# makgyver/rectorch

Hardware: AMD Instinct MI355X
Metric: MultiVAE train users/sec on ml-20m (synthetic, ml-20m-shaped) (higher is better)
Workload: dtype bf16

## Files before the change

### __graft_entry__.py

```python
import os
import subprocess
import sys

ROOT = os.path.dirname(os.path.abspath(__file__))
if ROOT not in sys.path:
    sys.path.insert(0, ROOT)


def build():
    from rectorch_amd import _lib
    path = _lib.build()
    assert os.path.exists(path)
    subprocess.check_call(["make", "-C", os.path.join(ROOT, "oracle"), "-s"])
    subprocess.check_call(["make", "-C", os.path.join(ROOT, "tests", "native"), "-s"])
    import rectorch_amd
    from rectorch_amd import nets, models, samplers, evaluation, metrics, parallel
    assert _lib.lib().rtx_abi_version() == 8


def smoke():
    import numpy as np
    import torch
    from scipy.sparse import csr_matrix
    from rectorch_amd.nets import MultiVAE_net
    from rectorch_amd.models import MultiVAE
    from rectorch_amd.samplers import DataSampler
    from rectorch_amd.utils import hash_state_dict
    from oracle import c_oracle

    assert torch.cuda.is_available(), "smoke() needs the MI355X"
    torch.cuda.set_device(0)
    I, H, L, B = 300, 64, 16, 24
    rng = np.random.default_rng(0)
    dense = (rng.random((B, I)) < 0.08).astype(np.float64)
    dense[3] = 0
    sd = hash_state_dict([I, H, L], [L, H, I], "vae", 7, bias_std=0.3)
    net = MultiVAE_net([L, H, I], dropout=0.5)
    net.load_state_dict({k: torch.from_numpy(v) for k, v in sd.items()})
    model = MultiVAE(net, beta=0.2, anneal_steps=0, numerics="fp32")
    smp = DataSampler(csr_matrix(dense), batch_size=B, shuffle=False)
    (rb,) = list(smp.iter_rows())
    mask = (rng.random((B, I)) >= 0.5).astype(np.uint8)
    eps = rng.standard_normal((B, L)).astype(np.float32)
    model._rtx.inject = (torch.from_numpy(mask).cuda(), torch.from_numpy(eps).cuda())
    loss = model._fused_step(rb, None, want_loss=True)
    params = [sd[k] for k in ["enc_layers.0.weight", "enc_layers.0.bias", "enc_layers.1.weight", "enc_layers.1.bias",
                              "dec_layers.0.weight", "dec_layers.0.bias", "dec_layers.1.weight", "dec_layers.1.bias"]]
# ... 17 lines not shown
```

### rectorch_amd/csrc/engine.hip

```cpp
#include "engine_internal.h"

int dev_alloc(rtx_engine* e, void** p, size_t bytes, bool zero)
{
    if (bytes == 0) bytes = 16;
    hipError_t rc = hipMalloc(p, bytes);
    if (rc != hipSuccess) {
        rtx_set_error("hipMalloc(%zu bytes) failed: %s", bytes, hipGetErrorString(rc));
        return RTX_ENOMEM;
    }
    if (e) e->allocs.push_back(*p);
    if (zero) {
        RTX_HIP(hipMemset(*p, 0, bytes));
        RTX_HIP(hipStreamSynchronize(nullptr));
    }
    return RTX_OK;
}

void dev_free(rtx_engine* e, void* p)
{
    if (!p) return;
    auto it = std::find(e->allocs.begin(), e->allocs.end(), p);
    if (it != e->allocs.end()) e->allocs.erase(it);
    (void)hipFree(p);
}
// ... 287 lines not shown
    const int Bp = rtx_pad_batch(B);
    static const rtx_step zero_step = {};
    if (!step) step = &zero_step;
    const int sample = training || e->gvae;
    int64_t in_chunks = 0;
    const bool sparse_in = l0 == 0 && l1 > 1 && sparse_in_ok(e, in, Bp, &in_chunks);
    if (l0 == 0) e->last_sparse_in = sparse_in;
    const bool gathered = e->gather_done;
    e->gather_done = false;
    if (e->join_fold && !(l0 == 0 && l1 > 1 && !sparse_in && gathered && e->bf16)) {
        e->join_fold = false;
        RTX_TRY(launch_hop_wait(e, st, 3, e->join_seq));
    }
    if (l0 == 0 && !sparse_in && !gathered) RTX_TRY(gather_batch(e, in, tg, B, training, step, st));
    for (int li = l0; li < l1; ++li) {
        Layer& l = e->L[li];
        if (li == e->NL - 1) {
            RtxGemm g = {};
            g.form = RTX_FORM_NT;
            g.A = l.A; g.B = l.Wsh; g.lda = l.inp; g.ldb = l.inp;
            g.k_slices = (int)((size_t)l.inp * e->esz / 128);
            g.splits = 1; g.C = logits; g.ldc = ldlog; g.bias = e->params[2 * li + 1];
            g.M_real = B; g.N_real = l.out;
            TIMED("gemm_logits");
            if (e->bf16 && !e->opt_nt_regstage) {
                g.tile_shape = (Bp % 512 == 0) ? RTX_DMA_512x128 : RTX_DMA_128x128;
                int bm, bn;
                rtx_gemm_dma_tile_dims(g.tile_shape, &bm, &bn);
                g.m_tiles = Bp / bm; g.n_tiles = l.outp / bn;
                if (want_lse && e->opt_lse_fuse) { g.lse_part = e->lse_part; g.lse_ld = e->lse_strips; }
                g.xcd_block = 1;
                RTX_TRY(rtx_gemm_dma_launch(g, RTX_EPI_BIAS_ROWS, st));
            } else {
                g.tile_shape = RTX_TILE_128x128;
                g.m_tiles = Bp / 128; g.n_tiles = l.outp / 128;
                if (want_lse && e->opt_lse_fuse) { g.lse_part = e->lse_part; g.lse_ld = e->lse_strips; }
                if (want_lse && logits16_on(e)) { g.C16 = l.D; g.ldc16 = l.outp; }
                RTX_TRY(rtx_gemm_launch(g, e->bf16 ? RTX_DT_BF16 : RTX_DT_F32, RTX_EPI_BIAS_ROWS, st));
            }
            break;
        }
        if (li == 0 && sparse_in) {
            RTX_TRY(ensure_in_chunks(e, in_chunks, st));
            RtxInChunksArgs c = {};
            c.in = *in; c.B = B; c.I = e->I; c.Iin = e->Iin;
            c.training = training; c.dropout_p = e->cfg.dropout_p;
            c.mask = step->dropout_mask; c.seed = step->seed; c.offset = step->offset;
            c.ent = e->in_ent; c.desc = e->in_desc; c.wsplit = e->in_wsplit; c.cap_chunks = e->in_cap_chunks;
            if (training) { c.target = *tg; c.tsum = e->tsum; c.X = (bf16_t*)l.A; c.ldx = l.inp; c.Bp = Bp; e->img_exact = false; }
            {
                TIMED("in_chunks");
                RTX_TRY(rtx_launch_in_chunks(c, st));
            }
            RtxSpmmInArgs a = {};
            a.ent = e->in_ent; a.desc = e->in_desc; a.wsplit = e->in_wsplit;
            a.B = B; a.Bp = Bp;
            a.W = (const bf16_t*)l.Wsh; a.ldw = l.inp; a.Kin = e->Iin;
            a.bias = e->params[2 * li + 1]; a.N_real = l.out; a.Np = l.outp; a.tanh_act = l.tanh_act;
            a.O32 = l.O32; a.R = (bf16_t*)e->L[li + 1].A; a.ones_col = 1;
            TIMED("spmm_in");
            RTX_TRY(rtx_launch_spmm_in(a, st));
            continue;
        }
        if (li > 0 && e->bf16 && e->opt_small_fwd && rtx_small_fwd_ok(l.inp)) {
            Layer& nx1 = e->L[li + 1];
            RtxSmallFwdArgs a = {};
            a.A = (const bf16_t*)l.A; a.W = (const bf16_t*)l.Wsh; a.lda = l.inp; a.ldw = l.inp; a.w_rows = l.outp;
            a.B = B; a.Bp = Bp; a.bias = e->params[2 * li + 1]; a.R = (bf16_t*)nx1.A;
// ... 592 lines not shown
```

### rectorch_amd/csrc/engine_api.hip

```cpp
#include "engine_internal.h"

extern "C" {

enum OptKind {
    OPT_BOOL,
    OPT_INT,
    OPT_CHECKED,
    OPT_COUNTER,
};
struct OptEntry {
    const char* key;
    OptKind kind;
    int rtx_engine::*member;
    int DpState::*dp_member;
};
static const OptEntry OPTIONS[] = {
    {"fuse_adam", OPT_BOOL, &rtx_engine::opt_fuse_adam},
    {"lse_fuse", OPT_BOOL, &rtx_engine::opt_lse_fuse},
    {"logits16", OPT_BOOL, &rtx_engine::opt_logits16},
    {"hop_values", OPT_BOOL, &rtx_engine::opt_hop_values},
    {"hop_kernels", OPT_BOOL, &rtx_engine::opt_hop_kernels},
    {"hop_fold", OPT_BOOL, &rtx_engine::opt_hop_fold},
    {"timing_calibrate", OPT_BOOL, &rtx_engine::opt_timing_calibrate},
    {"f32_dw_split", OPT_BOOL, &rtx_engine::opt_f32_dw_split},
    {"splitk_fwd", OPT_INT, &rtx_engine::opt_splitk_fwd},
    {"splitk_bwd", OPT_INT, &rtx_engine::opt_splitk_bwd},
    {"gather_scatter", OPT_BOOL, &rtx_engine::opt_gather_scatter},
    {"prefetch", OPT_BOOL, &rtx_engine::opt_prefetch},
    {"two_stream", OPT_BOOL, &rtx_engine::opt_two_stream},
    {"nt_regstage", OPT_BOOL, &rtx_engine::opt_nt_regstage},
    {"in_on_main", OPT_BOOL, &rtx_engine::opt_in_on_main},
    {"sparse_in", OPT_BOOL, &rtx_engine::opt_sparse_in},
    {"small_fwd", OPT_BOOL, &rtx_engine::opt_small_fwd},
    {"small_bwd", OPT_BOOL, &rtx_engine::opt_small_bwd},
    {"big_batch_tiles", OPT_BOOL, &rtx_engine::opt_big_batch_tiles},
    {"dw_side_pad", OPT_CHECKED, &rtx_engine::opt_dw_side_pad},
    {"dp_shard_min_elems", OPT_CHECKED, &rtx_engine::opt_dp_shard_min_elems},
    {"dp_one_comm", OPT_CHECKED, &rtx_engine::opt_dp_one_comm},
    {"dw_cfg", OPT_CHECKED, &rtx_engine::opt_dw_cfg},
    {"join_folds", OPT_COUNTER, &rtx_engine::st_join_folds},
    {"prefetch_hits", OPT_COUNTER, &rtx_engine::st_prefetch_hits},
    {"prefetch_issued", OPT_COUNTER, &rtx_engine::st_prefetch_issued},
    {"last_sparse_in", OPT_COUNTER, &rtx_engine::last_sparse_in},
    {"side_concurrent", OPT_COUNTER, &rtx_engine::side_concurrent},
    {"dp_collectives", OPT_COUNTER, nullptr, &DpState::st_collectives},
};
static const char* const OPTIONS_SET_ONLY = "hop_wrap, splitk, small_kw, small_waves";
static const char* const OPTIONS_GET_ONLY = "splitk, dp_bytes_all_reduce, dp_bytes_reduce_scatter, dp_bytes_all_gather, dp_two_comms";

static std::string option_keys(bool writable)
{
    std::string out;
    for (const OptEntry& o : OPTIONS)
        if (!writable || o.kind != OPT_COUNTER) out += std::string(o.key) + ", ";
    return out + (writable ? OPTIONS_SET_ONLY : OPTIONS_GET_ONLY);
}

static int set_checked(rtx_engine* e, const std::string& k, int32_t value, bool* handled)
{
    *handled = true;
    if (k == "dw_side_pad") e->opt_dw_side_pad = value > 0 ? value : 0;
    else if (k == "small_kw") rtx_small_set_kw(value);
    else if (k == "small_waves") rtx_small_set_waves(value);
// ... 197 lines not shown
```

### rectorch_amd/csrc/engine_internal.h

```cpp
#pragma once
#include "../../include/rectorch_hip.h"
#include "rtx_gemm.h"
#include "rtx_kernels.h"

#include <math.h>
#include <stdlib.h>
#include <string.h>
#include <sched.h>
#include <algorithm>
#include <chrono>
#include <map>
#include <string>
#include <vector>

const char* rtx_last_error_str();

struct Layer {
    int in = 0, out = 0, inp = 0, outp = 0;
    bool tanh_act = false;
    void* Wsh = nullptr;
    void* Wsh_alt = nullptr;
    void* WshT = nullptr;
    void* A = nullptr;
    float* O32 = nullptr;
// ... 85 lines not shown
    int opt_hop_values = 1;
    int n_cus = 256;
    int opt_f32_dw_split = 1;
    int opt_splitk_bwd = 0;
    int opt_splitk_fwd = 0;
    uint32_t* hopk_mem = nullptr;
    uint32_t hopk_seq = 0;
    bool join_pending = false, join_fold = false;
    uint32_t join_seq = 0;
    int opt_timing_calibrate = 0;
    int opt_dw_side_pad = 0;
    int opt_hop_fold = 1;
    int opt_hop_kernels = 0;
    uint32_t* hop_mem = nullptr;
    uint32_t hop_seq = 0;
    uint32_t hop_wrap = 0x7ffffff0u;
    int opt_fuse_adam = 1;
    int opt_dw_cfg = RTX_DW_64x128;
    int opt_dp_shard_min_elems = 1 << 20;
    uint32_t* loss_mailbox = nullptr;
    uint32_t loss_ticket = 0;
    int opt_dp_one_comm = 0;
    int opt_dw_cfg_set = 0;
    int opt_lse_fuse = 1;
    int opt_logits16 = 1;
    int opt_two_stream = 1;
    int opt_in_on_main = 1;
    int opt_sparse_in = 0;
    int opt_small_fwd = 1;
    int opt_small_bwd = 1;
    int opt_big_batch_tiles = 1;
    int last_sparse_in = 0;
    int opt_nt_regstage = 1;
    bool timing_all = false;
    std::map<std::string, int> timing_sites;
    std::map<std::string, long> timing_seen;
    std::map<std::string, TimingSite> sites;
    std::vector<hipEvent_t> event_pool;
    DpState dp;
};

struct ScopedTimer {
    rtx_engine* e;
    hipStream_t s;
    TimingSite* site = nullptr;
    hipEvent_t e0 = nullptr, e1 = nullptr;
    std::string name;
    ScopedTimer(rtx_engine* eng, const char* nm, hipStream_t st) : e(eng), s(st), name(nm)
    {
        const char* name = nm;
        if (!e->timing_all && e->timing_sites.empty()) return;
        if (!e->timing_all) {
            auto it = e->timing_sites.find(name);
            if (it == e->timing_sites.end()) return;
            if (it->second > 1 && (e->timing_seen[name]++ % it->second) != 0) return;
        }
        site = &e->sites[name];
        auto get = [&]() {
            hipEvent_t ev;
            if (!e->event_pool.empty()) {
                ev = e->event_pool.back();
                e->event_pool.pop_back();
            } else if (hipEventCreate(&ev) != hipSuccess) {
                ev = nullptr;
            }
            return ev;
// ... 82 lines not shown
```

### rectorch_amd/csrc/gemm.hip

```cpp
#include "rtx_gemm.h"
#include <type_traits>

typedef __attribute__((ext_vector_type(8))) __bf16 bf16x8_t;
typedef __attribute__((ext_vector_type(16))) float f32x16_t;

#define RTX_LDS_ROW_OF(KB) ((KB) + 16)

template <typename T> struct Mma;

template <> struct Mma<bf16_t> {
    static __device__ __forceinline__ void run(f32x16_t& acc, const uint4& a, const uint4& b)
    {
        acc = __builtin_amdgcn_mfma_f32_32x32x16_bf16(__builtin_bit_cast(bf16x8_t, a), __builtin_bit_cast(bf16x8_t, b),
                                                      acc, 0, 0, 0);
    }
};

template <> struct Mma<fp8_t> {
    static __device__ __forceinline__ void run(f32x16_t& acc, const uint4& a, const uint4& b)
    {
        const long a0 = (long)(((unsigned long)a.y << 32) | a.x), a1 = (long)(((unsigned long)a.w << 32) | a.z);
        const long b0 = (long)(((unsigned long)b.y << 32) | b.x), b1 = (long)(((unsigned long)b.w << 32) | b.z);
        acc = __builtin_amdgcn_mfma_f32_32x32x16_fp8_fp8(a0, b0, acc, 0, 0, 0);
        acc = __builtin_amdgcn_mfma_f32_32x32x16_fp8_fp8(a1, b1, acc, 0, 0, 0);
    }
};

template <> struct Mma<float> {
    static __device__ __forceinline__ void run(f32x16_t& acc, const uint4& a, const uint4& b)
    {
        acc = __builtin_amdgcn_mfma_f32_32x32x2f32(__builtin_bit_cast(float, a.x), __builtin_bit_cast(float, b.x), acc, 0, 0, 0);
        acc = __builtin_amdgcn_mfma_f32_32x32x2f32(__builtin_bit_cast(float, a.y), __builtin_bit_cast(float, b.y), acc, 0, 0, 0);
        acc = __builtin_amdgcn_mfma_f32_32x32x2f32(__builtin_bit_cast(float, a.z), __builtin_bit_cast(float, b.z), acc, 0, 0, 0);
        acc = __builtin_amdgcn_mfma_f32_32x32x2f32(__builtin_bit_cast(float, a.w), __builtin_bit_cast(float, b.w), acc, 0, 0, 0);
    }
};

template <int WM, int WN, int NB, int KB = 128> struct TileCfg {
    static constexpr int NT = WM * WN * 64;
    static constexpr int BM = WM * 64;
    static constexpr int BN = WN * NB * 32;
    static constexpr int LPR = KB / 16;
    static constexpr int RPP = NT / LPR;
    static constexpr int PA = BM / RPP;
    static constexpr int PB = BN / RPP;
    static constexpr int ROW = RTX_LDS_ROW_OF(KB);
    static constexpr int STAGE = (BM + BN) * ROW;
    static_assert(PA == 2 || PA == 4, "PA");
    static_assert(PB == 2 || PB == 4, "PB");
};

template <typename T, int EPI, int WM, int WN, int NB, int KB = 128, bool DEPTH3 = false>
__global__ __launch_bounds__(WM* WN * 64, KB == 64 ? 3 : ((WM * WN) / 4 > 2 ? (WM * WN) / 4 : 2)) void rtx_gemm_nt(const RtxGemm p)
{
    using Cfg = TileCfg<WM, WN, NB, KB>;
    constexpr int BM = Cfg::BM, BN = Cfg::BN, RPP = Cfg::RPP, PA = Cfg::PA, PB = Cfg::PB, STAGE = Cfg::STAGE;
    constexpr int RTX_LDS_ROW = Cfg::ROW, LPR_ST = Cfg::LPR;
    __shared__ __attribute__((aligned(16))) unsigned char smem[2 * STAGE];

    if (p.wait_word) rtx_fold_wait(p.wait_word, p.wait_seq);
    const int tid = threadIdx.x;
    const int lane = tid & 63, wave = tid >> 6;
    const int wm = wave / WN, wn = wave % WN;
    const int r = lane & 31, g = lane >> 5;

    int tm, tn, split;
    {
        const int L = blockIdx.x, xcd = L & 7, j = L >> 3;
        if (p.syrk_lower) {
            split = 0;
            const int patch = xcd + 8 * (j >> 6), within = j & 63;
            int pm = (int)((sqrtf(8.f * (float)patch + 1.f) - 1.f) * 0.5f);
            while ((pm + 1) * (pm + 2) / 2 <= patch) ++pm;
            while (pm * (pm + 1) / 2 > patch) --pm;
            const int pn = patch - pm * (pm + 1) / 2;
            tm = pm * 8 + (within & 7);
            tn = pn * 8 + (within >> 3);
            if (tm >= p.m_tiles || tn > tm) return;
        } else if (p.splits > 1) {
            const int tiles = p.m_tiles * p.n_tiles;
            split = xcd + 8 * (j / tiles);
            if (split >= p.splits) return;
            const int t = j % tiles;
            tm = t % p.m_tiles;
            tn = t / p.m_tiles;
        } else if (p.m_tiles <= p.n_tiles) {
            split = 0;
            tn = xcd + 8 * (j / p.m_tiles);
            tm = j % p.m_tiles;
            if (tn >= p.n_tiles) return;
        } else {
            split = 0;
            tm = xcd + 8 * (j / p.n_tiles);
            tn = j % p.n_tiles;
            if (tm >= p.m_tiles) return;
        }
    }
    const int k_sl = p.k_slices * (128 / KB);
    const int per = (k_sl + p.splits - 1) / p.splits;
    const int ks0 = split * per;
    const int ks1 = min(ks0 + per, k_sl);
    const int nk = ks1 - ks0;

    const size_t rowA = (size_t)p.lda * sizeof(T), rowB = (size_t)p.ldb * sizeof(T);
    const size_t kstA = p.a_slice_stride ? (size_t)p.a_slice_stride : (size_t)KB, kstB = p.b_slice_stride ? (size_t)p.b_slice_stride : (size_t)KB;
    const int st_row = tid / LPR_ST, st_ch = tid % LPR_ST;
    const unsigned char* gA = (const unsigned char*)p.A + ((size_t)tm * BM + st_row) * rowA + st_ch * 16;
    const unsigned char* gB = (const unsigned char*)p.B + ((size_t)tn * BN + st_row) * rowB + st_ch * 16;
    const int lds_a = st_row * RTX_LDS_ROW + st_ch * 16;
    const int lds_b = (BM + st_row) * RTX_LDS_ROW + st_ch * 16;

    uint4 ra0, ra1, ra2, ra3, rb0, rb1, rb2, rb3;
    uint4 sa0, sa1, sa2, sa3, sb0, sb1, sb2, sb3;
    f32x16_t acc[2][NB];
#pragma unroll
    for (int i = 0; i < 2; ++i)
#pragma unroll
        for (int j = 0; j < NB; ++j)
#pragma unroll
            for (int e = 0; e < 16; ++e) acc[i][j][e] = 0.f;

#define RTX_GL(R, X, q, base, row, ks) R##X##q = *(const uint4*)((base) + (size_t)(q) * RPP * (row) + (size_t)(ks) * ((row) == rowA ? kstA : kstB));
#define RTX_GLOAD(R, ks) {                                                  \
    RTX_GL(R, a, 0, gA, rowA, ks) RTX_GL(R, a, 1, gA, rowA, ks)             \
    if (PA == 4) { RTX_GL(R, a, 2, gA, rowA, ks) RTX_GL(R, a, 3, gA, rowA, ks) } \
    RTX_GL(R, b, 0, gB, rowB, ks) RTX_GL(R, b, 1, gB, rowB, ks)             \
    if (PB == 4) { RTX_GL(R, b, 2, gB, rowB, ks) RTX_GL(R, b, 3, gB, rowB, ks) } }
#define RTX_LS(R, X, q, off, st) *(uint4*)(smem + (st) * STAGE + (off) + (q) * RPP * RTX_LDS_ROW) = R##X##q;
#define RTX_LSTORE(R, st) {                                                 \
    RTX_LS(R, a, 0, lds_a, st) RTX_LS(R, a, 1, lds_a, st)                   \
    if (PA == 4) { RTX_LS(R, a, 2, lds_a, st) RTX_LS(R, a, 3, lds_a, st) }  \
    RTX_LS(R, b, 0, lds_b, st) RTX_LS(R, b, 1, lds_b, st)                   \
    if (PB == 4) { RTX_LS(R, b, 2, lds_b, st) RTX_LS(R, b, 3, lds_b, st) } }
#define RTX_COMPUTE(st)                                                                                       \
    {                                                                                                         \
        const unsigned char* sA = smem + (st) * STAGE + (wm * 64 + r) * RTX_LDS_ROW + g * 16;                 \
        const unsigned char* sB = smem + (st) * STAGE + (BM + wn * (NB * 32) + r) * RTX_LDS_ROW + g * 16;     \
        _Pragma("unroll") for (int kk = 0; kk < KB / 32; ++kk) {                                              \
            const uint4 a0 = *(const uint4*)(sA + kk * 32);                                                   \
            const uint4 a1 = *(const uint4*)(sA + 32 * RTX_LDS_ROW + kk * 32);                                \
            _Pragma("unroll") for (int j = 0; j < NB; ++j) {                                                  \
                const uint4 b = *(const uint4*)(sB + j * 32 * RTX_LDS_ROW + kk * 32);                         \
                Mma<T>::run(acc[0][j], a0, b);                                                                \
                Mma<T>::run(acc[1][j], a1, b);                                                                \
            }                                                                                                 \
        }                                                                                                     \
    }

    if constexpr (DEPTH3) {
        uint4 ua0, ua1, ua2, ua3, ub0, ub1, ub2, ub3;
        if (nk > 0) {
            RTX_GLOAD(r, ks0)
            RTX_LSTORE(r, 0)
            RTX_GLOAD(r, min(ks0 + 1, ks1 - 1))
            RTX_GLOAD(s, min(ks0 + 2, ks1 - 1))
            __syncthreads();
#define RTX_STEP(U, R, st, k)                                                   \
            RTX_GLOAD(U, min(ks0 + t + (k) + 3, ks1 - 1))                       \
            __builtin_amdgcn_sched_barrier(0);                                  \
            if (t + (k) < nk) { RTX_COMPUTE(st) }                               \
            if (t + (k) + 1 < nk) { RTX_LSTORE(R, 1 - (st)) }                   \
            __syncthreads();
            for (int t = 0; t < nk; t += 6) {
                RTX_STEP(u, r, 0, 0) RTX_STEP(r, s, 1, 1) RTX_STEP(s, u, 0, 2)
                RTX_STEP(u, r, 1, 3) RTX_STEP(r, s, 0, 4) RTX_STEP(s, u, 1, 5)
            }
#undef RTX_STEP
        }
    } else if (nk == 1) {
        RTX_GLOAD(r, ks0)
        RTX_LSTORE(r, 0)
        __syncthreads();
        RTX_COMPUTE(0)
    } else if (nk > 1) {
        RTX_GLOAD(r, ks0)
        RTX_LSTORE(r, 0)
        RTX_GLOAD(r, ks0 + 1)
        __syncthreads();
        int t = 0;
        for (; t + 3 < nk; t += 2) {
            RTX_GLOAD(s, ks0 + t + 2)
            __builtin_amdgcn_sched_barrier(0);
            RTX_COMPUTE(0)
            RTX_LSTORE(r, 1)
            __syncthreads();
            RTX_GLOAD(r, ks0 + t + 3)
            __builtin_amdgcn_sched_barrier(0);
            RTX_COMPUTE(1)
            RTX_LSTORE(s, 0)
            __syncthreads();
        }
        const bool three = (nk - t) == 3;
        if (three) { RTX_GLOAD(s, ks0 + t + 2) }
        RTX_COMPUTE(0)
        RTX_LSTORE(r, 1)
        __syncthreads();
        RTX_COMPUTE(1)
        if (three) {
            RTX_LSTORE(s, 0)
            __syncthreads();
            RTX_COMPUTE(0)
        }
    }
#undef RTX_GL
#undef RTX_GLOAD
#undef RTX_LS
#undef RTX_LSTORE
#undef RTX_COMPUTE

    if constexpr (EPI == RTX_EPI_BIAS_ROWS) {
        typedef __attribute__((ext_vector_type(4))) float f32x4_t;
        constexpr int WCOLS = NB * 32, WLD = WCOLS + 4, HC = WCOLS / 2, NQ = HC / 4;
        static_assert(WM * WN * 32 * WLD * 4 <= 2 * STAGE, "epilogue scratch must fit in the stages");
        __syncthreads();
        float* wreg = (float*)smem + wave * (32 * WLD);
        const int erow = lane >> 1, ehalf = lane & 1;
        constexpr int LPR = WCOLS / 4, RPI = 64 / LPR;
        const int srow = lane / LPR, scol = (lane % LPR) * 4;
        const int col0 = tn * BN + wn * WCOLS;
        float bj[NB];
#pragma unroll
        for (int j = 0; j < NB; ++j) {
            const int col = col0 + j * 32 + r;
            bj[j] = p.bias ? p.bias[col < p.N_real ? col : 0] : 0.f;
        }
        const long ld = p.ldc;
        const bool vec_ok = ((ld & 3) == 0) && (((uintptr_t)p.C & 15) == 0);
#pragma unroll
        for (int i = 0; i < 2; ++i) {
#pragma unroll
            for (int j = 0; j < NB; ++j)
#pragma unroll
                for (int e = 0; e < 16; ++e) wreg[((e & 3) + 8 * (e >> 2) + 4 * g) * WLD + j * 32 + r] = acc[i][j][e] + bj[j];
            __builtin_amdgcn_wave_barrier();
            f32x4_t v[NQ];
#pragma unroll
            for (int q = 0; q < NQ; ++q) v[q] = *(const f32x4_t*)(wreg + erow * WLD + ehalf * HC + q * 4);
            __builtin_amdgcn_wave_barrier();
            const int row = tm * BM + wm * 64 + i * 32 + erow;
            const int colh = col0 + ehalf * HC;
            if (p.lse_part) {
                float m = -INFINITY;
#pragma unroll
                for (int q = 0; q < NQ; ++q)
#pragma unroll
                    for (int k = 0; k < 4; ++k)
                        if (colh + q * 4 + k < p.N_real) m = fmaxf(m, v[q][k]);
                const float mm = fmaxf(m, __shfl_xor(m, 1, 64));
                float sum = 0.f;
                if (mm != -INFINITY) {
#pragma unroll
                    for (int q = 0; q < NQ; ++q)
#pragma unroll
                        for (int k = 0; k < 4; ++k)
                            if (colh + q * 4 + k < p.N_real) sum += __expf(v[q][k] - mm);
                }
                sum += __shfl_xor(sum, 1, 64);
                if (ehalf == 0 && row < p.M_real) p.lse_part[(size_t)row * p.lse_ld + (tn * WN + wn)] = make_float2(mm, sum);
            }
            f32x4_t w[32 / RPI];
#pragma unroll
            for (int it = 0; it < 32 / RPI; ++it) w[it] = *(const f32x4_t*)(wreg + (it * RPI + srow) * WLD + scol);
            __builtin_amdgcn_wave_barrier();
            if (p.C16) {
                typedef __attribute__((ext_vector_type(4))) _Float16 f16x4_t;
#pragma unroll
                for (int it = 0; it < 32 / RPI; ++it) {
                    const int orow = tm * BM + wm * 64 + i * 32 + it * RPI + srow;
                    if (orow < p.M_real) {
                        f16x4_t h;
#pragma unroll
                        for (int k = 0; k < 4; ++k) h[k] = (_Float16)__builtin_amdgcn_fmed3f(w[it][k], -65504.f, 65504.f);
                        *(f16x4_t*)((_Float16*)p.C16 + (size_t)orow * p.ldc16 + col0 + scol) = h;
                    }
                }
                continue;
            }
#pragma unroll
            for (int it = 0; it < 32 / RPI; ++it) {
                const int orow = tm * BM + wm * 64 + i * 32 + it * RPI + srow;
                const int c = col0 + scol;
                if (orow < p.M_real) {
                    float* dst = p.C + (size_t)orow * ld + c;
                    if (vec_ok && c + 3 < p.N_real) {
                        *(f32x4_t*)dst = w[it];
                    } else {
#pragma unroll
                        for (int k = 0; k < 4; ++k)
                            if (c + k < p.N_real) dst[k] = w[it][k];
                    }
                }
            }
        }
        return;
    }
    const int row_base = tm * BM + wm * 64 + 4 * g;
    const int col_base = tn * BN + wn * (NB * 32) + r;
    const long ld = (EPI == RTX_EPI_GRAD) ? (long)p.N_real : p.ldc;
    float* cp = p.C + (EPI == RTX_EPI_STORE ? (size_t)split * p.slab_stride : (size_t)0) + (size_t)row_base * ld + col_base;
#pragma unroll
    for (int i = 0; i < 2; ++i) {
#pragma unroll
        for (int j = 0; j < NB; ++j) {
            const int col = col_base + j * 32;
#pragma unroll
            for (int e = 0; e < 16; ++e) {
                const int dr = i * 32 + (e & 3) + 8 * (e >> 2);
                const int row = row_base + dr;
                const float v = acc[i][j][e];
                float* dst = cp + (long)dr * ld + j * 32;
                if (EPI == RTX_EPI_STORE) {
                    *dst = v;
                } else {
                    if (row < p.M_real) {
                        if (col < p.N_real)
                            *dst = v;
                        else if (col == p.N_real && p.gbias)
                            p.gbias[row] = v;
                    }
                }
            }
        }
    }
}

struct TileShape {
    int wm, wn, nb, kb;
    bool depth3;
    unsigned epis[3];
    const char* only;
};
constexpr unsigned EPI_S = 1u << RTX_EPI_STORE, EPI_B = 1u << RTX_EPI_BIAS_ROWS, EPI_G = 1u << RTX_EPI_GRAD, EPI_ALL = EPI_S | EPI_B | EPI_G;
constexpr TileShape kTile[RTX_TILE_COUNT] = {
     {2, 2, 2, 128, false, {EPI_ALL, EPI_ALL, EPI_S}, nullptr},
     {4, 2, 2, 128, false, {EPI_ALL, EPI_ALL, 0}, nullptr},
     {2, 4, 2, 128, false, {EPI_ALL, EPI_ALL, 0}, nullptr},
     {2, 2, 2, 64, false, {0, EPI_B, 0}, "the 64-byte-slice tile exists for bf16 operands with the bias epilogue only"},
     {2, 2, 2, 128, true, {0, EPI_S | EPI_B, 0}, "the depth-3 tile exists for bf16 operands with the store / bias epilogues only"},
};

void rtx_gemm_tile_dims(int shape, int* bm, int* bn)
{
    const TileShape& t = kTile[shape >= 0 && shape < RTX_TILE_COUNT ? shape : RTX_TILE_128x128];
    *bm = t.wm * 64;
    *bn = t.wn * t.nb * 32;
}

template <typename T> constexpr int kDtypeOf = std::is_same<T, float>::value ? RTX_DT_F32 : std::is_same<T, bf16_t>::value ? RTX_DT_BF16 : RTX_DT_FP8;

template <typename T, int EPI> static void launch_shape(const RtxGemm& g, dim3 grid, hipStream_t stream)
{
    rtx_dispatch_index<RTX_TILE_COUNT>(g.tile_shape, [&](auto shape) {
        constexpr TileShape t = kTile[decltype(shape)::value];
        if constexpr ((t.epis[kDtypeOf<T>] >> EPI) & 1)
            hipLaunchKernelGGL((rtx_gemm_nt<T, EPI, t.wm, t.wn, t.nb, t.kb, t.depth3>), grid, dim3(t.wm * t.wn * 64), 0, stream, g);
    });
}

template <typename T> static void launch_type(const RtxGemm& g, int epilogue, dim3 grid, hipStream_t stream)
{
    rtx_dispatch_index<3>(epilogue, [&](auto epi) { launch_shape<T, decltype(epi)::value>(g, grid, stream); });
}

int rtx_gemm_launch(const RtxGemm& g, int dtype, int epilogue, hipStream_t stream)
{
    RTX_CHECK(dtype >= RTX_DT_F32 && dtype <= RTX_DT_FP8, RTX_EINVAL, "gemm: bad operand type %d", dtype);
    RTX_CHECK(epilogue >= RTX_EPI_STORE && epilogue <= RTX_EPI_GRAD, RTX_EINVAL, "gemm: bad epilogue %d", epilogue);
    RTX_CHECK(g.tile_shape >= 0 && g.tile_shape < RTX_TILE_COUNT, RTX_EINVAL, "gemm: bad tile shape %d", g.tile_shape);
    const TileShape& tile = kTile[g.tile_shape];
    const bool served = (tile.epis[dtype] >> epilogue) & 1;
    RTX_CHECK(dtype != RTX_DT_FP8 || served, RTX_EINVAL,
              "gemm: fp8 operands only with the plain-store epilogue and the 128x128 tile (Gram matrix of binary data)");
    RTX_CHECK(served, RTX_EINVAL, "gemm: %s", tile.only);
    RTX_CHECK(g.m_tiles > 0 && g.n_tiles > 0 && g.k_slices > 0 && g.splits > 0, RTX_EINVAL, "gemm: empty problem");
    RTX_CHECK(epilogue == RTX_EPI_STORE || g.splits == 1, RTX_EINVAL, "gemm: split-K only with EPI_STORE");
    if (g.C16) {
        RTX_CHECK(epilogue == RTX_EPI_BIAS_ROWS && dtype == RTX_DT_BF16 && (g.ldc16 & 3) == 0 && (((uintptr_t)g.C16) & 7) == 0 &&
                      g.ldc16 >= (long)g.n_tiles * (tile.wn * tile.nb * 32),
                  RTX_EINVAL, "gemm: half-precision logits need the bias epilogue, bf16 operands and an 8-byte aligned [M][ldc16 >= N_pad] image");
    }
    const int tiles = g.m_tiles * g.n_tiles;
    int groups, gsize;
    if (g.syrk_lower) {
        RTX_CHECK(g.m_tiles == g.n_tiles && g.splits == 1 && g.tile_shape == RTX_TILE_128x128 && epilogue == RTX_EPI_STORE, RTX_EINVAL,
                  "gemm: syrk_lower needs a square 128x128-tiled problem without split-K");
        const int pr = (g.m_tiles + 7) / 8;
        groups = pr * (pr + 1) / 2;
        gsize = 64;
    } else if (g.splits > 1) { groups = g.splits; gsize = tiles; }
    else if (g.m_tiles <= g.n_tiles) { groups = g.n_tiles; gsize = g.m_tiles; }
    else { groups = g.m_tiles; gsize = g.n_tiles; }
    const dim3 grid((unsigned)(8 * ((groups + 7) / 8) * gsize));
    if (dtype == RTX_DT_FP8) launch_type<fp8_t>(g, epilogue, grid, stream);
    else if (dtype == RTX_DT_BF16) launch_type<bf16_t>(g, epilogue, grid, stream);
    else launch_type<float>(g, epilogue, grid, stream);
    RTX_HIP(hipGetLastError());
    return RTX_OK;
}
```

### rectorch_amd/csrc/rtx_gemm.h

```cpp
#pragma once
#include "rtx_common.h"
#include <type_traits>
#include <utility>

template <typename F, int... Is> static inline bool rtx_dispatch_index_impl(int index, F& f, std::integer_sequence<int, Is...>)
{
    return ((index == Is && (f(std::integral_constant<int, Is>{}), true)) || ...);
}
template <int N, typename F> static inline bool rtx_dispatch_index(int index, F&& f)
{
    return rtx_dispatch_index_impl(index, f, std::make_integer_sequence<int, N>{});
}

enum RtxEpilogue {
    RTX_EPI_STORE = 0,
    RTX_EPI_BIAS_ROWS = 1,
    RTX_EPI_GRAD = 2,
};

struct RtxAdamEpi {
    float* p;
    float* m;
    float* v;
    float* gkeep;
    void* sh;
    void* shT;
    int ld_sh, ld_shT;
    float step_size, bc2_sqrt, beta1, beta2, eps, weight_decay;
    float lam;
    const float* sumsq;
};

enum RtxTileShape {
    RTX_TILE_128x128 = 0,
    RTX_TILE_256x128 = 1,
    RTX_TILE_128x256 = 2,
    RTX_TILE_128x128_K32 = 3,
    RTX_TILE_128x128_D3 = 4,
    RTX_TILE_COUNT
};
void rtx_gemm_tile_dims(int shape, int* bm, int* bn);

enum RtxForm { RTX_FORM_NT = 0, RTX_FORM_NN = 1, RTX_FORM_TN = 2 };
enum RtxDmaCfg { RTX_DMA_128x128 = 0, RTX_DMA_512x128 = 1, RTX_DMA_256x256 = 2, RTX_DMA_128x128_S2 = 3, RTX_DMA_256x256_W4 = 4, RTX_DMA_256x256_LW = 5 };
void rtx_gemm_dma_tile_dims(int cfg, int* bm, int* bn);

struct RtxGemm {
    const void* A;
    const void* B;
    int form;
    long lda, ldb;
    long a_slice_stride, b_slice_stride;
    int tile_shape;
    int m_tiles, n_tiles;
    int k_slices;
    int splits;
    int syrk_lower;
    float* C;
    long ldc;
    long slab_stride;
    const float* bias;
    float* gbias;
    int M_real, N_real;
    float2* lse_part;
    int lse_ld;
    void* C16;
    long ldc16;
    int xcd_block;
    unsigned* hop_word;
    unsigned hop_seq;
    const unsigned* wait_word;
    unsigned wait_seq;
};

enum RtxDtype { RTX_DT_F32 = 0, RTX_DT_BF16 = 1, RTX_DT_FP8 = 2 };

int rtx_gemm_launch(const RtxGemm& g, int dtype, int epilogue, hipStream_t stream);
int rtx_gemm_dma_launch(const RtxGemm& g, int epilogue, hipStream_t stream);

int rtx_gemm_f32_km_launch(const RtxGemm& g, int epilogue, hipStream_t stream);

enum RtxDwEpilogue { RTX_DW_GRAD = 0, RTX_DW_ADAM = 1 };
enum RtxDwCfg {
    RTX_DW_64x128 = 0,
    RTX_DW_32x128 = 1,
    RTX_DW_32x128_S2 = 2,
    RTX_DW_128x128 = 3,
    RTX_DW_128x128_W4 = 4,
    RTX_DW_32x256 = 5,
    RTX_DW_32x256_S3 = 6,
    RTX_DW_32x256_K32 = 7,
    RTX_DW_128x128_K32 = 8,
    RTX_DW_CFG_COUNT
};
struct RtxDw {
    const void* A;
    const void* B;
    long lda, ldb;
    int m_tiles, n_tiles;
    int k_slices;
    int M_real, N_real;
    float* gW;
    bf16_t* g16;
    float* gbias;
    bf16_t* gbias16;
    RtxAdamEpi adam;
    float* bias_p;
    float* bias_m;
    float* bias_v;
    const float* bias_sumsq;
// ... 17 lines not shown
```

Baseline: 1.932 million.

## Add swizzled 128x192 NT GEMM tile for logits with wave-count heuristic

Adds a wide 128x192 tile variant to the register-staged NT GEMM, with an XOR-swizzled, unpadded LDS layout and a guarded last tile that may cover a partial width. The logits GEMM picks it through a heuristic: use it when the 128x128 tile count exceeds two blocks per CU but the 192-wide tile count fits. The goal is fewer tail waves and more B-operand reuse per block on the large output projection. The risks are extra register pressure from six B staging registers and more epilogue complexity. LSE partial indexing now keys on 64-column strips.

```diff
diff --git a/__graft_entry__.py b/__graft_entry__.py
--- a/__graft_entry__.py
+++ b/__graft_entry__.py
@@ -13,6 +13,7 @@
     assert os.path.exists(path)
     subprocess.check_call(["make", "-C", os.path.join(ROOT, "oracle"), "-s"])
     subprocess.check_call(["make", "-C", os.path.join(ROOT, "tests", "native"), "-s"])
+    subprocess.check_call(["make", "-C", os.path.join(ROOT, "tests", "native"), "-f", "wide.mk", "-s"])
     import rectorch_amd
     from rectorch_amd import nets, models, samplers, evaluation, metrics, parallel
     assert _lib.lib().rtx_abi_version() == 8
diff --git a/rectorch_amd/csrc/engine.hip b/rectorch_amd/csrc/engine.hip
--- a/rectorch_amd/csrc/engine.hip
+++ b/rectorch_amd/csrc/engine.hip
@@ -343,8 +343,11 @@
                 g.xcd_block = 1;
                 RTX_TRY(rtx_gemm_dma_launch(g, RTX_EPI_BIAS_ROWS, st));
             } else {
-                g.tile_shape = RTX_TILE_128x128;
-                g.m_tiles = Bp / 128; g.n_tiles = l.outp / 128;
+                g.tile_shape = !e->bf16 ? RTX_TILE_128x128 : e->opt_logits_tile == 0 ? RTX_TILE_128x128 : e->opt_logits_tile == 1 ? RTX_TILE_128x192
+                                                           : rtx_gemm_logits_tile(Bp, l.outp, e->n_cus);
+                int bm, bn;
+                rtx_gemm_tile_dims(g.tile_shape, &bm, &bn);
+                g.m_tiles = Bp / bm; g.n_tiles = (l.outp + bn - 1) / bn; g.n_pad = l.outp;
                 if (want_lse && e->opt_lse_fuse) { g.lse_part = e->lse_part; g.lse_ld = e->lse_strips; }
                 if (want_lse && logits16_on(e)) { g.C16 = l.D; g.ldc16 = l.outp; }
                 RTX_TRY(rtx_gemm_launch(g, e->bf16 ? RTX_DT_BF16 : RTX_DT_F32, RTX_EPI_BIAS_ROWS, st));
diff --git a/rectorch_amd/csrc/engine_api.hip b/rectorch_amd/csrc/engine_api.hip
--- a/rectorch_amd/csrc/engine_api.hip
+++ b/rectorch_amd/csrc/engine_api.hip
@@ -29,6 +29,7 @@
     {"prefetch", OPT_BOOL, &rtx_engine::opt_prefetch},
     {"two_stream", OPT_BOOL, &rtx_engine::opt_two_stream},
     {"nt_regstage", OPT_BOOL, &rtx_engine::opt_nt_regstage},
+    {"logits_tile", OPT_INT, &rtx_engine::opt_logits_tile},
     {"in_on_main", OPT_BOOL, &rtx_engine::opt_in_on_main},
     {"sparse_in", OPT_BOOL, &rtx_engine::opt_sparse_in},
     {"small_fwd", OPT_BOOL, &rtx_engine::opt_small_fwd},
diff --git a/rectorch_amd/csrc/engine_internal.h b/rectorch_amd/csrc/engine_internal.h
--- a/rectorch_amd/csrc/engine_internal.h
+++ b/rectorch_amd/csrc/engine_internal.h
@@ -141,6 +141,7 @@
     int opt_big_batch_tiles = 1;
     int last_sparse_in = 0;
     int opt_nt_regstage = 1;
+    int opt_logits_tile = -1;
     bool timing_all = false;
     std::map<std::string, int> timing_sites;
     std::map<std::string, long> timing_seen;
diff --git a/rectorch_amd/csrc/gemm.hip b/rectorch_amd/csrc/gemm.hip
--- a/rectorch_amd/csrc/gemm.hip
+++ b/rectorch_amd/csrc/gemm.hip
@@ -5,6 +5,7 @@
 typedef __attribute__((ext_vector_type(16))) float f32x16_t;
 
 #define RTX_LDS_ROW_OF(KB) ((KB) + 16)
+#define RTX_LDS_SWZ(row, chunk) ((((chunk) ^ (((row) >> 1) & 7))) * 16)
 
 template <typename T> struct Mma;
 
@@ -36,25 +37,28 @@
     }
 };
 
-template <int WM, int WN, int NB, int KB = 128> struct TileCfg {
+template <int WM, int WN, int NB, int KB = 128, bool WIDE = false> struct TileCfg {
+    static constexpr int MB = WIDE ? 1 : 2;
     static constexpr int NT = WM * WN * 64;
-    static constexpr int BM = WM * 64;
+    static constexpr int BM = WM * MB * 32;
     static constexpr int BN = WN * NB * 32;
     static constexpr int LPR = KB / 16;
     static constexpr int RPP = NT / LPR;
     static constexpr int PA = BM / RPP;
     static constexpr int PB = BN / RPP;
-    static constexpr int ROW = RTX_LDS_ROW_OF(KB);
+    static constexpr int ROW = WIDE ? KB : RTX_LDS_ROW_OF(KB);
     static constexpr int STAGE = (BM + BN) * ROW;
     static_assert(PA == 2 || PA == 4, "PA");
-    static_assert(PB == 2 || PB == 4, "PB");
-};
-
-template <typename T, int EPI, int WM, int WN, int NB, int KB = 128, bool DEPTH3 = false>
+    static_assert(PB == 2 || PB == 4 || PB == 6, "PB");
+    static_assert(!WIDE || (KB == 128 && RPP == 32 && BM % 16 == 0), "the swizzle key (row >> 1) & 7 must not change from pass to pass");
+};
+
+template <typename T, int EPI, int WM, int WN, int NB, int KB = 128, bool DEPTH3 = false, bool WIDE = false>
 __global__ __launch_bounds__(WM* WN * 64, KB == 64 ? 3 : ((WM * WN) / 4 > 2 ? (WM * WN) / 4 : 2)) void rtx_gemm_nt(const RtxGemm p)
 {
-    using Cfg = TileCfg<WM, WN, NB, KB>;
-    constexpr int BM = Cfg::BM, BN = Cfg::BN, RPP = Cfg::RPP, PA = Cfg::PA, PB = Cfg::PB, STAGE = Cfg::STAGE;
+    using Cfg = TileCfg<WM, WN, NB, KB, WIDE>;
+    static_assert(!WIDE || (EPI == RTX_EPI_BIAS_ROWS && !DEPTH3), "the wide tile's last tile is guarded in the logits epilogue only");
+    constexpr int MB = Cfg::MB, BM = Cfg::BM, BN = Cfg::BN, RPP = Cfg::RPP, PA = Cfg::PA, PB = Cfg::PB, STAGE = Cfg::STAGE;
     constexpr int RTX_LDS_ROW = Cfg::ROW, LPR_ST = Cfg::LPR;
     __shared__ __attribute__((aligned(16))) unsigned char smem[2 * STAGE];
 
@@ -107,48 +111,65 @@
     const int st_row = tid / LPR_ST, st_ch = tid % LPR_ST;
     const unsigned char* gA = (const unsigned char*)p.A + ((size_t)tm * BM + st_row) * rowA + st_ch * 16;
     const unsigned char* gB = (const unsigned char*)p.B + ((size_t)tn * BN + st_row) * rowB + st_ch * 16;
-    const int lds_a = st_row * RTX_LDS_ROW + st_ch * 16;
-    const int lds_b = (BM + st_row) * RTX_LDS_ROW + st_ch * 16;
-
-    uint4 ra0, ra1, ra2, ra3, rb0, rb1, rb2, rb3;
-    uint4 sa0, sa1, sa2, sa3, sb0, sb1, sb2, sb3;
-    f32x16_t acc[2][NB];
-#pragma unroll
-    for (int i = 0; i < 2; ++i)
+    const int st_slot = WIDE ? RTX_LDS_SWZ(st_row, st_ch) : st_ch * 16;
+    const int lds_a = st_row * RTX_LDS_ROW + st_slot;
+    const int lds_b = (BM + st_row) * RTX_LDS_ROW + st_slot;
+    size_t bq[6] = {};
+    if constexpr (WIDE) {
+        const int b_pass = min(PB, (p.n_pad - tn * BN) / RPP);
+#pragma unroll
+        for (int q = 0; q < PB; ++q) bq[q] = (size_t)(q < b_pass ? q : 0) * RPP * rowB;
+    }
+    int slk[4] = {};
+    if constexpr (WIDE) {
+#pragma unroll
+        for (int kk = 0; kk < 4; ++kk) slk[kk] = RTX_LDS_SWZ(r, g + 2 * kk);
+    }
+
+    uint4 ra0, ra1, ra2, ra3, rb0, rb1, rb2, rb3, rb4, rb5;
+    uint4 sa0, sa1, sa2, sa3, sb0, sb1, sb2, sb3, sb4, sb5;
+    f32x16_t acc[MB][NB];
+#pragma unroll
+    for (int i = 0; i < MB; ++i)
 #pragma unroll
         for (int j = 0; j < NB; ++j)
 #pragma unroll
             for (int e = 0; e < 16; ++e) acc[i][j][e] = 0.f;
 
-#define RTX_GL(R, X, q, base, row, ks) R##X##q = *(const uint4*)((base) + (size_t)(q) * RPP * (row) + (size_t)(ks) * ((row) == rowA ? kstA : kstB));
+#define RTX_GLA(R, q, ks) R##a##q = *(const uint4*)(gA + (size_t)(q) * RPP * rowA + (size_t)(ks) * kstA);
+#define RTX_GLB(R, q, ks) R##b##q = *(const uint4*)(gB + (WIDE ? bq[q] : (size_t)(q) * RPP * rowB) + (size_t)(ks) * kstB);
 #define RTX_GLOAD(R, ks) {                                                  \
-    RTX_GL(R, a, 0, gA, rowA, ks) RTX_GL(R, a, 1, gA, rowA, ks)             \
-    if (PA == 4) { RTX_GL(R, a, 2, gA, rowA, ks) RTX_GL(R, a, 3, gA, rowA, ks) } \
-    RTX_GL(R, b, 0, gB, rowB, ks) RTX_GL(R, b, 1, gB, rowB, ks)             \
-    if (PB == 4) { RTX_GL(R, b, 2, gB, rowB, ks) RTX_GL(R, b, 3, gB, rowB, ks) } }
+    RTX_GLA(R, 0, ks) RTX_GLA(R, 1, ks)                                     \
+    if (PA == 4) { RTX_GLA(R, 2, ks) RTX_GLA(R, 3, ks) }                    \
+    RTX_GLB(R, 0, ks) RTX_GLB(R, 1, ks)                                     \
+    if (PB >= 4) { RTX_GLB(R, 2, ks) RTX_GLB(R, 3, ks) }                    \
+    if (PB == 6) { RTX_GLB(R, 4, ks) RTX_GLB(R, 5, ks) } }
 #define RTX_LS(R, X, q, off, st) *(uint4*)(smem + (st) * STAGE + (off) + (q) * RPP * RTX_LDS_ROW) = R##X##q;
 #define RTX_LSTORE(R, st) {                                                 \
     RTX_LS(R, a, 0, lds_a, st) RTX_LS(R, a, 1, lds_a, st)                   \
     if (PA == 4) { RTX_LS(R, a, 2, lds_a, st) RTX_LS(R, a, 3, lds_a, st) }  \
     RTX_LS(R, b, 0, lds_b, st) RTX_LS(R, b, 1, lds_b, st)                   \
-    if (PB == 4) { RTX_LS(R, b, 2, lds_b, st) RTX_LS(R, b, 3, lds_b, st) } }
+    if (PB >= 4) { RTX_LS(R, b, 2, lds_b, st) RTX_LS(R, b, 3, lds_b, st) }  \
+    if (PB == 6) { RTX_LS(R, b, 4, lds_b, st) RTX_LS(R, b, 5, lds_b, st) } }
 #define RTX_COMPUTE(st)                                                                                       \
     {                                                                                                         \
-        const unsigned char* sA = smem + (st) * STAGE + (wm * 64 + r) * RTX_LDS_ROW + g * 16;                 \
-        const unsigned char* sB = smem + (st) * STAGE + (BM + wn * (NB * 32) + r) * RTX_LDS_ROW + g * 16;     \
+        const unsigned char* sA = smem + (st) * STAGE + (wm * (MB * 32) + r) * RTX_LDS_ROW + (WIDE ? 0 : g * 16);             \
+        const unsigned char* sB = smem + (st) * STAGE + (BM + wn * (NB * 32) + r) * RTX_LDS_ROW + (WIDE ? 0 : g * 16);        \
         _Pragma("unroll") for (int kk = 0; kk < KB / 32; ++kk) {                                              \
-            const uint4 a0 = *(const uint4*)(sA + kk * 32);                                                   \
-            const uint4 a1 = *(const uint4*)(sA + 32 * RTX_LDS_ROW + kk * 32);                                \
+            const int ko = WIDE ? slk[kk & 3] : kk * 32;                                                      \
+            const uint4 a0 = *(const uint4*)(sA + ko);                                                        \
+            uint4 a1 = a0;                                                                                    \
+            if constexpr (MB == 2) a1 = *(const uint4*)(sA + 32 * RTX_LDS_ROW + ko);                          \
             _Pragma("unroll") for (int j = 0; j < NB; ++j) {                                                  \
-                const uint4 b = *(const uint4*)(sB + j * 32 * RTX_LDS_ROW + kk * 32);                         \
+                const uint4 b = *(const uint4*)(sB + j * 32 * RTX_LDS_ROW + ko);                              \
                 Mma<T>::run(acc[0][j], a0, b);                                                                \
-                Mma<T>::run(acc[1][j], a1, b);                                                                \
+                if constexpr (MB == 2) Mma<T>::run(acc[MB - 1][j], a1, b);                                    \
             }                                                                                                 \
         }                                                                                                     \
     }
 
     if constexpr (DEPTH3) {
-        uint4 ua0, ua1, ua2, ua3, ub0, ub1, ub2, ub3;
+        uint4 ua0, ua1, ua2, ua3, ub0, ub1, ub2, ub3, ub4, ub5;
         if (nk > 0) {
             RTX_GLOAD(r, ks0)
             RTX_LSTORE(r, 0)
@@ -202,7 +223,8 @@
             RTX_COMPUTE(0)
         }
     }
-#undef RTX_GL
+#undef RTX_GLA
+#undef RTX_GLB
 #undef RTX_GLOAD
 #undef RTX_LS
 #undef RTX_LSTORE
@@ -210,34 +232,39 @@
 
     if constexpr (EPI == RTX_EPI_BIAS_ROWS) {
         typedef __attribute__((ext_vector_type(4))) float f32x4_t;
-        constexpr int WCOLS = NB * 32, WLD = WCOLS + 4, HC = WCOLS / 2, NQ = HC / 4;
+        static_assert(NB % 2 == 0, "a wave owns whole 64-column strips");
+        constexpr int NS = NB / 2, WCOLS = 64, WLD = WCOLS + 4, HC = WCOLS / 2, NQ = HC / 4;
         static_assert(WM * WN * 32 * WLD * 4 <= 2 * STAGE, "epilogue scratch must fit in the stages");
         __syncthreads();
         float* wreg = (float*)smem + wave * (32 * WLD);
         const int erow = lane >> 1, ehalf = lane & 1;
         constexpr int LPR = WCOLS / 4, RPI = 64 / LPR;
         const int srow = lane / LPR, scol = (lane % LPR) * 4;
-        const int col0 = tn * BN + wn * WCOLS;
+        const int wcol0 = tn * BN + wn * (NB * 32);
         float bj[NB];
 #pragma unroll
         for (int j = 0; j < NB; ++j) {
-            const int col = col0 + j * 32 + r;
+            const int col = wcol0 + j * 32 + r;
             bj[j] = p.bias ? p.bias[col < p.N_real ? col : 0] : 0.f;
         }
         const long ld = p.ldc;
         const bool vec_ok = ((ld & 3) == 0) && (((uintptr_t)p.C & 15) == 0);
 #pragma unroll
-        for (int i = 0; i < 2; ++i) {
-#pragma unroll
-            for (int j = 0; j < NB; ++j)
-#pragma unroll
-                for (int e = 0; e < 16; ++e) wreg[((e & 3) + 8 * (e >> 2) + 4 * g) * WLD + j * 32 + r] = acc[i][j][e] + bj[j];
+        for (int i = 0; i < MB; ++i)
+#pragma unroll
+        for (int s = 0; s < NS; ++s) {
+            const int col0 = wcol0 + s * WCOLS;
+            if (WIDE && col0 >= p.n_pad) continue;
+#pragma unroll
+            for (int j = 0; j < 2; ++j)
+#pragma unroll
+                for (int e = 0; e < 16; ++e) wreg[((e & 3) + 8 * (e >> 2) + 4 * g) * WLD + j * 32 + r] = acc[i][2 * s + j][e] + bj[2 * s + j];
             __builtin_amdgcn_wave_barrier();
             f32x4_t v[NQ];
 #pragma unroll
             for (int q = 0; q < NQ; ++q) v[q] = *(const f32x4_t*)(wreg + erow * WLD + ehalf * HC + q * 4);
             __builtin_amdgcn_wave_barrier();
-            const int row = tm * BM + wm * 64 + i * 32 + erow;
+            const int row = tm * BM + wm * (MB * 32) + i * 32 + erow;
             const int colh = col0 + ehalf * HC;
             if (p.lse_part) {
                 float m = -INFINITY;
@@ -256,7 +283,7 @@
                             if (colh + q * 4 + k < p.N_real) sum += __expf(v[q][k] - mm);
                 }
                 sum += __shfl_xor(sum, 1, 64);
-                if (ehalf == 0 && row < p.M_real) p.lse_part[(size_t)row * p.lse_ld + (tn * WN + wn)] = make_float2(mm, sum);
+                if (ehalf == 0 && row < p.M_real) p.lse_part[(size_t)row * p.lse_ld + (col0 >> 6)] = make_float2(mm, sum);
             }
             f32x4_t w[32 / RPI];
 #pragma unroll
@@ -266,7 +293,7 @@
                 typedef __attribute__((ext_vector_type(4))) _Float16 f16x4_t;
 #pragma unroll
                 for (int it = 0; it < 32 / RPI; ++it) {
-                    const int orow = tm * BM + wm * 64 + i * 32 + it * RPI + srow;
+                    const int orow = tm * BM + wm * (MB * 32) + i * 32 + it * RPI + srow;
                     if (orow < p.M_real) {
                         f16x4_t h;
 #pragma unroll
@@ -278,7 +305,7 @@
             }
 #pragma unroll
             for (int it = 0; it < 32 / RPI; ++it) {
-                const int orow = tm * BM + wm * 64 + i * 32 + it * RPI + srow;
+                const int orow = tm * BM + wm * (MB * 32) + i * 32 + it * RPI + srow;
                 const int c = col0 + scol;
                 if (orow < p.M_real) {
                     float* dst = p.C + (size_t)orow * ld + c;
@@ -294,12 +321,12 @@
         }
         return;
     }
-    const int row_base = tm * BM + wm * 64 + 4 * g;
+    const int row_base = tm * BM + wm * (MB * 32) + 4 * g;
     const int col_base = tn * BN + wn * (NB * 32) + r;
     const long ld = (EPI == RTX_EPI_GRAD) ? (long)p.N_real : p.ldc;
     float* cp = p.C + (EPI == RTX_EPI_STORE ? (size_t)split * p.slab_stride : (size_t)0) + (size_t)row_base * ld + col_base;
 #pragma unroll
-    for (int i = 0; i < 2; ++i) {
+    for (int i = 0; i < MB; ++i) {
 #pragma unroll
         for (int j = 0; j < NB; ++j) {
             const int col = col_base + j * 32;
@@ -326,24 +353,32 @@
 
 struct TileShape {
     int wm, wn, nb, kb;
-    bool depth3;
+    bool depth3, wide;
     unsigned epis[3];
     const char* only;
 };
 constexpr unsigned EPI_S = 1u << RTX_EPI_STORE, EPI_B = 1u << RTX_EPI_BIAS_ROWS, EPI_G = 1u << RTX_EPI_GRAD, EPI_ALL = EPI_S | EPI_B | EPI_G;
 constexpr TileShape kTile[RTX_TILE_COUNT] = {
-     {2, 2, 2, 128, false, {EPI_ALL, EPI_ALL, EPI_S}, nullptr},
-     {4, 2, 2, 128, false, {EPI_ALL, EPI_ALL, 0}, nullptr},
-     {2, 4, 2, 128, false, {EPI_ALL, EPI_ALL, 0}, nullptr},
-     {2, 2, 2, 64, false, {0, EPI_B, 0}, "the 64-byte-slice tile exists for bf16 operands with the bias epilogue only"},
-     {2, 2, 2, 128, true, {0, EPI_S | EPI_B, 0}, "the depth-3 tile exists for bf16 operands with the store / bias epilogues only"},
+     {2, 2, 2, 128, false, false, {EPI_ALL, EPI_ALL, EPI_S}, nullptr},
+     {4, 2, 2, 128, false, false, {EPI_ALL, EPI_ALL, 0}, nullptr},
+     {2, 4, 2, 128, false, false, {EPI_ALL, EPI_ALL, 0}, nullptr},
+     {2, 2, 2, 64, false, false, {0, EPI_B, 0}, "the 64-byte-slice tile exists for bf16 operands with the bias epilogue only"},
+     {2, 2, 2, 128, true, false, {0, EPI_S | EPI_B, 0}, "the depth-3 tile exists for bf16 operands with the store / bias epilogues only"},
+     {4, 1, 6, 128, false, true, {0, EPI_B, 0}, "the 128 x 192 tile exists for bf16 operands with the bias epilogue only"},
 };
 
 void rtx_gemm_tile_dims(int shape, int* bm, int* bn)
 {
     const TileShape& t = kTile[shape >= 0 && shape < RTX_TILE_COUNT ? shape : RTX_TILE_128x128];
-    *bm = t.wm * 64;
+    *bm = t.wm * (t.wide ? 32 : 64);
     *bn = t.wn * t.nb * 32;
+}
+
+int rtx_gemm_logits_tile(int Mp, int Np, int n_cus)
+{
+    const long slots = 2L * n_cus;
+    const long t128 = (long)(Mp / 128) * (Np / 128), t192 = (long)(Mp / 128) * ((Np + 191) / 192);
+    return t128 > slots && t192 <= slots ? RTX_TILE_128x192 : RTX_TILE_128x128;
 }
 
 template <typename T> constexpr int kDtypeOf = std::is_same<T, float>::value ? RTX_DT_F32 : std::is_same<T, bf16_t>::value ? RTX_DT_BF16 : RTX_DT_FP8;
@@ -353,17 +388,35 @@
     rtx_dispatch_index<RTX_TILE_COUNT>(g.tile_shape, [&](auto shape) {
         constexpr TileShape t = kTile[decltype(shape)::value];
         if constexpr ((t.epis[kDtypeOf<T>] >> EPI) & 1)
-            hipLaunchKernelGGL((rtx_gemm_nt<T, EPI, t.wm, t.wn, t.nb, t.kb, t.depth3>), grid, dim3(t.wm * t.wn * 64), 0, stream, g);
+            hipLaunchKernelGGL((rtx_gemm_nt<T, EPI, t.wm, t.wn, t.nb, t.kb, t.depth3, t.wide>), grid, dim3(t.wm * t.wn * 64), 0, stream, g);
     });
 }
 
+int rtx_gemm_resident_per_cu(int shape, int epilogue, int* out)
+{
+    RTX_CHECK(shape >= 0 && shape < RTX_TILE_COUNT && epilogue >= RTX_EPI_STORE && epilogue <= RTX_EPI_GRAD && out, RTX_EINVAL, "gemm: bad tile shape / epilogue");
+    RTX_CHECK((kTile[shape].epis[RTX_DT_BF16] >> epilogue) & 1, RTX_EINVAL, "gemm: %s", kTile[shape].only);
+    hipError_t rc = hipSuccess;
+    rtx_dispatch_index<RTX_TILE_COUNT>(shape, [&](auto sh) {
+        rtx_dispatch_index<3>(epilogue, [&](auto epi) {
+            constexpr TileShape t = kTile[decltype(sh)::value];
+            constexpr int EPI = decltype(epi)::value;
+            if constexpr ((t.epis[RTX_DT_BF16] >> EPI) & 1)
+                rc = hipOccupancyMaxActiveBlocksPerMultiprocessor(out, rtx_gemm_nt<bf16_t, EPI, t.wm, t.wn, t.nb, t.kb, t.depth3, t.wide>, t.wm * t.wn * 64, 0);
+        });
+    });
+    RTX_HIP(rc);
+    return RTX_OK;
+}
+
 template <typename T> static void launch_type(const RtxGemm& g, int epilogue, dim3 grid, hipStream_t stream)
 {
     rtx_dispatch_index<3>(epilogue, [&](auto epi) { launch_shape<T, decltype(epi)::value>(g, grid, stream); });
 }
 
-int rtx_gemm_launch(const RtxGemm& g, int dtype, int epilogue, hipStream_t stream)
-{
+int rtx_gemm_launch(const RtxGemm& g_in, int dtype, int epilogue, hipStream_t stream)
+{
+    RtxGemm g = g_in;
     RTX_CHECK(dtype >= RTX_DT_F32 && dtype <= RTX_DT_FP8, RTX_EINVAL, "gemm: bad operand type %d", dtype);
     RTX_CHECK(epilogue >= RTX_EPI_STORE && epilogue <= RTX_EPI_GRAD, RTX_EINVAL, "gemm: bad epilogue %d", epilogue);
     RTX_CHECK(g.tile_shape >= 0 && g.tile_shape < RTX_TILE_COUNT, RTX_EINVAL, "gemm: bad tile shape %d", g.tile_shape);
@@ -374,9 +427,13 @@
     RTX_CHECK(served, RTX_EINVAL, "gemm: %s", tile.only);
     RTX_CHECK(g.m_tiles > 0 && g.n_tiles > 0 && g.k_slices > 0 && g.splits > 0, RTX_EINVAL, "gemm: empty problem");
     RTX_CHECK(epilogue == RTX_EPI_STORE || g.splits == 1, RTX_EINVAL, "gemm: split-K only with EPI_STORE");
+    const int bn = tile.wn * tile.nb * 32;
+    if (g.n_pad == 0) g.n_pad = g.n_tiles * bn;
+    RTX_CHECK(g.n_pad == g.n_tiles * bn || (tile.wide && g.n_pad % 64 == 0 && g.n_pad > (g.n_tiles - 1) * bn && g.n_pad < g.n_tiles * bn), RTX_EINVAL,
+              "gemm: n_pad = %d must be the tiles' %d columns (128 x 192 tile: a multiple of 64 inside the last tile)", g.n_pad, g.n_tiles * bn);
     if (g.C16) {
         RTX_CHECK(epilogue == RTX_EPI_BIAS_ROWS && dtype == RTX_DT_BF16 && (g.ldc16 & 3) == 0 && (((uintptr_t)g.C16) & 7) == 0 &&
-                      g.ldc16 >= (long)g.n_tiles * (tile.wn * tile.nb * 32),
+                      g.ldc16 >= (long)g.n_pad,
                   RTX_EINVAL, "gemm: half-precision logits need the bias epilogue, bf16 operands and an 8-byte aligned [M][ldc16 >= N_pad] image");
     }
     const int tiles = g.m_tiles * g.n_tiles;
diff --git a/rectorch_amd/csrc/rtx_gemm.h b/rectorch_amd/csrc/rtx_gemm.h
--- a/rectorch_amd/csrc/rtx_gemm.h
+++ b/rectorch_amd/csrc/rtx_gemm.h
@@ -37,9 +37,11 @@
     RTX_TILE_128x256 = 2,
     RTX_TILE_128x128_K32 = 3,
     RTX_TILE_128x128_D3 = 4,
+    RTX_TILE_128x192 = 5,
     RTX_TILE_COUNT
 };
 void rtx_gemm_tile_dims(int shape, int* bm, int* bn);
+int rtx_gemm_logits_tile(int Mp, int Np, int n_cus);
 
 enum RtxForm { RTX_FORM_NT = 0, RTX_FORM_NN = 1, RTX_FORM_TN = 2 };
 enum RtxDmaCfg { RTX_DMA_128x128 = 0, RTX_DMA_512x128 = 1, RTX_DMA_256x256 = 2, RTX_DMA_128x128_S2 = 3, RTX_DMA_256x256_W4 = 4, RTX_DMA_256x256_LW = 5 };
@@ -71,11 +73,13 @@
     unsigned hop_seq;
     const unsigned* wait_word;
     unsigned wait_seq;
+    int n_pad;
 };
 
 enum RtxDtype { RTX_DT_F32 = 0, RTX_DT_BF16 = 1, RTX_DT_FP8 = 2 };
 
 int rtx_gemm_launch(const RtxGemm& g, int dtype, int epilogue, hipStream_t stream);
+int rtx_gemm_resident_per_cu(int shape, int epilogue, int* out);
 int rtx_gemm_dma_launch(const RtxGemm& g, int epilogue, hipStream_t stream);
 
 int rtx_gemm_f32_km_launch(const RtxGemm& g, int epilogue, hipStream_t stream);
```

Result: no change. 1.957 million, median of 3 (+1.3%).
